# OSU-Bee-Lab/buzzdetect

Hardware: AMD Instinct MI355X
Metric: yamnet_windows_per_s (higher is better)
Workload: dtype f32 (split-f16x3 MFMA products, f32 accumulate)

## Files before the change

### buzzdetect_amd/csrc/bd_device.h

```cpp
#pragma once

#include "bd_internal.h"

#include <mutex>
#include <type_traits>
#ifdef BD_KERNEL_TRACE
#include <cstdio>
#include <cstdlib>
#endif

namespace bd {

namespace {

typedef float f32x16 __attribute__((ext_vector_type(16)));
typedef float v2f __attribute__((ext_vector_type(2)));
typedef float v4f __attribute__((ext_vector_type(4)));
typedef unsigned v4u __attribute__((ext_vector_type(4)));
typedef unsigned u32x2 __attribute__((ext_vector_type(2)));
typedef _Float16 f16x2 __attribute__((ext_vector_type(2)));
typedef _Float16 f16x4 __attribute__((ext_vector_type(4)));
typedef _Float16 f16x8 __attribute__((ext_vector_type(8)));

constexpr float kF16Max = 65504.0f;
// ... 71 lines not shown
                    }
    return true;
}
static_assert(tr_image_is_bijection(), "every (half, k, chunk) has its own 8 bytes of the slot, and they fill it");
static_assert(tr_image_writes_conflict_free(), "a lane group of the publication meets no bank twice");
static_assert(tr_image_reads_conflict_free(), "a lane half of the transposed read meets no bank twice");
__device__ __forceinline__ int tr_read_lane_off(int lane) {
    const int g = lane >> 4, q = (lane >> 2) & 3, p = lane & 3;
    return tr_image_off(0, tr_read_k(0, g >> 1, 0, q), tr_read_chunk(0, g & 1, p));
}
__host__ __device__ constexpr int tr_read_next(int off) { return (off ^ 16) + 4 * kTrRowBytes; }
constexpr bool tr_read_next_holds() {
    for (int lane = 0; lane < 64; ++lane) {
        const int g = lane >> 4, q = (lane >> 2) & 3, p = lane & 3;
        if (tr_read_next(tr_image_off(0, tr_read_k(0, g >> 1, 0, q), tr_read_chunk(0, g & 1, p))) !=
            tr_image_off(0, tr_read_k(0, g >> 1, 1, q), tr_read_chunk(0, g & 1, p)))
            return false;
        for (int s = 0; s < 2; ++s)
            for (int i = 0; i < 3; ++i)
                for (int r = 0; r < 2; ++r)
                    if (tr_image_off(0, tr_read_k(s, g >> 1, r, q), tr_read_chunk(i, g & 1, p)) !=
                        tr_image_off(0, tr_read_k(0, g >> 1, r, q), tr_read_chunk(0, g & 1, p)) + 16 * s * kTrRowBytes + 64 * i)
                        return false;
    }
    return true;
}
static_assert(tr_read_next_holds(), "the reader's immediates");
__device__ __forceinline__ f16x8 tr_read_frag(const char* p0, const char* p1) {
    typedef short s16x4 __attribute__((ext_vector_type(4)));
    typedef __attribute__((address_space(3))) s16x4* lds4;
    const s16x4 a = __builtin_amdgcn_ds_read_tr16_b64_v4i16((lds4)p0), b = __builtin_amdgcn_ds_read_tr16_b64_v4i16((lds4)p1);
    return __builtin_bit_cast(f16x8, __builtin_shufflevector(a, b, 0, 1, 2, 3, 4, 5, 6, 7));
}

__device__ __forceinline__ unsigned pw_lds_addr(const void* p) {
    return (unsigned)(unsigned long long)(__attribute__((address_space(3))) const void*)p;
}
template <int OFFSET>
__device__ __forceinline__ f16x8 pw_lds_frag(unsigned addr) {
    f16x8 v;
    asm volatile("ds_read_b128 %0, %1 offset:%2" : "=v"(v) : "v"(addr), "n"(OFFSET) : "memory");
    return v;
}
__device__ __forceinline__ void pw_lds_store64(unsigned addr, f16x4 v) {
    asm volatile("ds_write_b64 %0, %1" ::"v"(addr), "v"(v) : "memory");
}
__device__ __forceinline__ f16x8 pw_landed(f16x8 v) {
    asm volatile("" : "+v"(v));
    return v;
}
template <int N>
__device__ __forceinline__ void pw_lds_wait() {
    asm volatile("s_waitcnt lgkmcnt(%0)" ::"n"(N) : "memory");
}
template <int I, int E, typename F>
__device__ __forceinline__ void static_for_pw(F&& f) {
    if constexpr (I < E) {
        f(std::integral_constant<int, I>{});
        static_for_pw<I + 1, E>(f);
    }
}
template <int K16, int V, int R>
struct PwResSchedule {
    static constexpr int split_at(int q) {
        for (int j = 0; j < V; ++j)
            if (q == j * K16 / (V > 0 ? V : 1) + 1) return j;
// ... 59 lines not shown
```

### buzzdetect_amd/csrc/bd_internal.h

```cpp
#pragma once

#include <hip/hip_runtime.h>
#include <stdint.h>

#include <string>
#include <vector>

#include "../../include/buzzdetect_hip.h"

namespace bd {

constexpr int kMelNonZero = 461;

constexpr int kMelStart[BD_MEL_BANDS] = {
    5, 5, 6, 7, 9, 10, 11, 12, 13, 14, 16, 17, 18, 20, 21, 23, 25, 26, 28, 30, 32, 34, 36, 38, 40, 42, 44, 47, 49, 52, 54, 57,
    60, 63, 66, 69, 72, 76, 79, 83, 87, 90, 95, 99, 103, 108, 112, 117, 122, 127, 133, 138, 144, 150, 156, 162, 169, 176, 183,
    190, 198, 206, 214, 223};
constexpr int kMelLen[BD_MEL_BANDS] = {
    1, 2, 3, 3, 2, 2, 2, 2, 3, 3, 2, 3, 3, 3, 4, 3, 3, 4, 4, 4, 4, 4, 4, 4, 4, 5, 5, 5, 5, 5, 6, 6,
    6, 6, 6, 7, 7, 7, 8, 7, 8, 9, 8, 9, 9, 9, 10, 10, 11, 11, 11, 12, 12, 12, 13, 14, 14, 14, 15, 16, 16, 17, 17, 17};
constexpr int mel_offset(int band) {
    int o = 0;
    for (int m = 0; m < band; ++m) o += kMelLen[m];
    return o;
// ... 138 lines not shown
                                  hipStream_t stream);
bool launch_separable_fused_next_dw(const float* in, float* out, int windows, const SepLayer& L, const SepLayer& next,
                                    hipStream_t stream);
void launch_pool_head(const float* act, int windows, const float* head_wt, const float* head_b,
                      int n_classes, float* emb, float* logits, hipStream_t stream);
void launch_head(const float* pooled, int windows, const float* head_wt, const float* head_b, int n_classes,
                 float* logits, hipStream_t stream);

void launch_pointwise_res(const float* in, float* out, int rows, const SepLayer& L, hipStream_t stream);
void launch_pointwise_sep_ws(const float* in, float* out, int64_t rows, const SepLayer& L, hipStream_t stream);
bool launch_sep_ws_next_dw(const float* in, float* out, int windows, const SepLayer& L, const SepLayer& next, hipStream_t stream);

bool launch_l4_window_next_dw(const float* in, float* out, int windows, const SepLayer& L, const SepLayer& next, hipStream_t stream);
bool l4_window_planes_supported(const SepLayer& L3, const SepLayer& L4, const SepLayer& L5);
bool launch_l4_window_planes(const void* planes, const SepLayer& L3, const SepLayer& L4, const SepLayer& L5, float* out,
                             int windows, hipStream_t stream);

void launch_stem4(const float* logmel, int patch_step, const WindowMap& map, int w0, int windows, const float* c1_w,
                  const float* c1_b,
                  const SepLayer& L2, const SepLayer& L3, float* out, hipStream_t stream);

void launch_stem_reg(const float* logmel, int patch_step, const WindowMap& map, int w0, int windows, const float* c1_w,
                     const float* c1_b, const SepLayer& L2, const SepLayer& L3, float* out, hipStream_t stream);
void launch_stem_reg_planes(const float* logmel, int patch_step, const WindowMap& map, int w0, int windows, const float* c1_w,
                            const float* c1_b, const SepLayer& L2, const SepLayer& L3, float* out, hipStream_t stream);

void launch_stem_reg_f32(const float* logmel, int patch_step, const WindowMap& map, int w0, int windows, const float* c1_w,
                         const float* c1_b, const SepLayer& L2, const SepLayer& L3, float* out, hipStream_t stream);

bool launch_l4_reg_f32(const float* in, float* out, int windows, const SepLayer& L4, const SepLayer& L5, hipStream_t stream);

bool launch_separable_mid(const float* in, float* out, int windows, const SepLayer& L5, const SepLayer& L6, const SepLayer& L7,
                          hipStream_t stream);
constexpr int kDw7PlaneBytes = 8 * 2 * 24 * 32 * 2;
bool separable_mid_planes_supported(const SepLayer& L5, const SepLayer& L6, const SepLayer& L7);
bool launch_separable_mid_planes(const float* in, void* out, int windows, const SepLayer& L5, const SepLayer& L6, const SepLayer& L7,
                                 hipStream_t stream);

bool launch_separable_mid_f32(const float* in, float* out, int windows, const SepLayer& L5, const SepLayer& L6, const SepLayer& L7,
                              hipStream_t stream);

bool separable_chip_pw7_supported(const SepLayer& L7, const SepLayer* L, int nl, const SepLayer& next, int windows);
bool launch_separable_chip_pw7(const void* in, float* out, int windows, const SepLayer& L7, const SepLayer* L, int nl,
                               const SepLayer& next, hipStream_t stream);
int launch_separable_run_next_dw(const float* a, float* b, int windows, const SepLayer* L, int max_layers, hipStream_t stream,
                                 bool planes = false);

bool launch_separable_chip_f32(const float* in, float* out, int windows, const SepLayer* L, int nl, hipStream_t stream,
                               const SepLayer* next, bool dw0_done);

bool tail_supported(const SepLayer& L13, const SepLayer& L14);
bool launch_tail_pw13_dw14(const void* in, void* out, int windows, const SepLayer& L13, const SepLayer& L14, hipStream_t stream);
bool launch_tail_pw14_pool(const void* in, float* pooled, int windows, const SepLayer& L14, hipStream_t stream);
bool tail_f32_supported(const SepLayer& L13, const SepLayer& L14);
bool launch_tail_f32(const float* in, float* mid, float* pooled, int windows, const SepLayer& L13, const SepLayer& L14, hipStream_t stream,
                     int which);

struct DenseLayer {
    int k, n;
    int act;
    const float* wfrag;
    const float* bias;
};
size_t dense_packed_floats(int k, int n);
void dense_pack_weights(const float* kernel, int k, int n, float* dst);
void launch_dense(const float* A, int lda, int windows, const DenseLayer& L, float* C, int ldc, hipStream_t stream);
void launch_softmax_rows(const float* x, int ldx, float* y, int windows, int n, hipStream_t stream);
// ... 52 lines not shown
```

### buzzdetect_amd/csrc/sepchip.hip

```cpp
#include "bd_device.h"

namespace bd {

namespace {

constexpr int kChipHalfBytes = 97 * 64;
constexpr int kChipSlotBytes = 2 * kChipHalfBytes;

constexpr int kChipMaxLayers = 5;
struct ChipChain {
    const float* dw_w[kChipMaxLayers];
    const float* dw_b[kChipMaxLayers];
    const _Float16* whi[kChipMaxLayers];
    const _Float16* wlo[kChipMaxLayers];
    const float* pw_u[kChipMaxLayers];
    const float* pw_b[kChipMaxLayers];
    const float* ndw_w;
    const _Float16 *w7hi, *w7lo;
    const float *u7, *b7;
};
template <typename T>
__device__ __forceinline__ const T* chain_ptr(int field, int li) {
    typedef const __attribute__((address_space(4))) unsigned long long* kptr;
    const kptr ka = (kptr)__builtin_amdgcn_kernarg_segment_ptr();
    return reinterpret_cast<const T*>(ka[field * kChipMaxLayers + li]);
}
static_assert(sizeof(ChipChain) == (6 * kChipMaxLayers + 5) * 8, "six tables of five pointers + five");

template <bool PLAIN, int NSLOT, bool TRACE = false, bool NDW = false, bool PLANES = false, bool PW7 = false>
__global__ __launch_bounds__(512, 2) void sep_chip_kernel(const ChipChain ch, const float* X, float* Y, int nl,
                                                           long long M, unsigned* __restrict__ range_flag,
                                                           unsigned long long* __restrict__ dbg = nullptr, int tune = 0) {
    static_assert(NSLOT >= 9 && NSLOT <= 16, "ring size");
    constexpr int K = 512, KQ = K / 16;
    constexpr int NPEND = 16 - NSLOT;
    extern __shared__ __attribute__((aligned(16))) char sm[];
    const int tid = threadIdx.x;
    const int lane = tid & 63;
    const int wc = __builtin_amdgcn_readfirstlane(tid >> 6);
    const int frow = lane & 31, fh = lane >> 5;
    const long long m0 = (long long)blockIdx.x * 96;
    float rmax = 0.0f;
    int tsn = 0;
#define CHIP_TS()                                                                                         \
    if constexpr (TRACE) {                                                                                \
        if (blockIdx.x == 0 && lane == 0 && (wc == 0 || wc == 5) && tsn < 64)                             \
            dbg[(wc == 5 ? 64 : 0) + tsn] = __builtin_amdgcn_s_memtime();                                 \
        ++tsn;                                                                                            \
    }
    CHIP_TS()

    const int wk0 = ((frow >> 1) & 7) << 3;
    const int ra0 = frow * 64 + ((fh ^ ((frow >> 2) & 3)) << 4);
    const int ra1 = ra0 + 2048 + (frow >= 16 ? 64 : 0);
    const int rt0 = tr_read_lane_off(lane), rt1 = tr_read_next(rt0);
    const unsigned lane16 = lane * 16, c4 = frow * 4;

    f32x16 acc[3][2];
    unsigned pend[48], out0[48];

#define CHIP_DW(J, ST, TAPS)                                                                              \
    {                                                                                                     \
        float wt[9];                                                                                      \
        _Pragma("unroll") for (int t = 0; t < 9; ++t)                                                     \
            wt[t] = __builtin_bit_cast(float, __builtin_amdgcn_raw_buffer_load_b32(TAPS, c4, (t * K + 32 * (ST)) * 4, 0)); \
        const float shift = __builtin_bit_cast(float, __builtin_amdgcn_raw_buffer_load_b32(TAPS, c4, (9 * K + 32 * (ST)) * 4, 0)); \
        _Pragma("unroll") for (int y = 0; y < 6; ++y)                                                     \
            _Pragma("unroll") for (int xp = 0; xp < 2; ++xp) {                                            \
                v2f a[2];                                                                                 \
                _Pragma("unroll") for (int d = 0; d < 2; ++d) {                                           \
                    const int x = 2 * xp + d;                                                             \
                    a[d] = v2f{shift, shift};                                                             \
                    _Pragma("unroll") for (int kh = 0; kh < 3; ++kh)                                      \
                        _Pragma("unroll") for (int kw = 0; kw < 3; ++kw) {                                \
                            const int iy = y + kh - 1, ix = x + kw - 1;                                   \
                            if (iy < 0 || iy >= 6 || ix < 0 || ix >= 4) continue;                         \
                            a[d] = __builtin_elementwise_fma(in2[iy][ix], v2f{wt[kh * 3 + kw], wt[kh * 3 + kw]}, a[d]); \
                        }                                                                                 \
                }                                                                                         \
                _Pragma("unroll") for (int w = 0; w < 2; ++w) {                                           \
                    const float v0 = fmaxf(w ? a[0].y : a[0].x, 0.0f), v1 = fmaxf(w ? a[1].y : a[1].x, 0.0f); \
                    const f16x2 h_ = {(_Float16)v0, (_Float16)v1};     \
                    const unsigned hi_ = __builtin_bit_cast(unsigned, h_);                                \
                    unsigned lo_;                                                                         \
                     \
                     \
                    asm volatile("v_fma_mixlo_f16 %0, %2, -1.0, %3 op_sel:[0,0,0] op_sel_hi:[1,0,0]\n\t"  \
                                 "v_fma_mixhi_f16 %0, %2, -1.0, %4 op_sel:[1,0,0] op_sel_hi:[1,0,0]\n\t"  \
                                 "v_max_f32 %1, %1, %3\n\tv_max_f32 %1, %1, %4"                           \
                                 : "=&v"(lo_), "+v"(rmax) : "v"(hi_), "v"(v0), "v"(v1));                  \
                    const int ci = 2 * (6 * w + y) + xp;     \
                    if ((J) == 1) { pend[ci] = hi_; pend[24 + ci] = lo_; }                                \
                    else { out0[ci] = hi_; out0[24 + ci] = lo_; }                                         \
                }                                                                                         \
            }                                                                                             \
    }
#define CHIP_PUBLISH()                                                                                    \
    {                                                                                                     \
        int wkl = wk0;        \
        asm volatile("" : "+v"(wkl));                             \
        char* const slot0 = sm + wc * kChipSlotBytes + frow * kTrRowBytes;                                \
        _Pragma("unroll") for (int j = 0; j < 12; ++j) CHIP_PUT(slot0, j, out0)                           \
        if (wc + 8 < NSLOT) {                                                \
            char* const slot1 = sm + (wc + 8) * kChipSlotBytes + frow * kTrRowBytes;                      \
            _Pragma("unroll") for (int j = 0; j < 12; ++j) CHIP_PUT(slot1, j, pend)                       \
        }                                                                                                 \
    }
#define CHIP_PUT(ROW, J, PK)                                                                              \
    {                                                                                                     \
        char* const p_ = (ROW) + ((96 * fh + 8 * (J)) ^ wkl);                                             \
        *reinterpret_cast<u32x2*>(p_) = u32x2{PK[2 * (J)], PK[2 * (J) + 1]};                              \
        *reinterpret_cast<u32x2*>(p_ + kTrHalfBytes) = u32x2{PK[24 + 2 * (J)], PK[25 + 2 * (J)]};         \
    }
#define CHIP_TAPS_RSRC(DW_W) __builtin_amdgcn_make_buffer_rsrc(const_cast<float*>(DW_W), 0, 10 * K * 4, 0x00020000)

    auto k_loop = [&](auto kq_c, auto row_c, const _Float16* const Wfhi, const _Float16* const Wflo) __attribute__((always_inline)) {
        constexpr int KQL = decltype(kq_c)::value;
        constexpr bool ROWIMG = decltype(row_c)::value;
        constexpr int NS = KQL / 2;
        constexpr int NP = NS > NSLOT ? NS - NSLOT : 0;
        static_assert(NP == 0 || NP == NPEND, "a layer of K = 512 or one that fits the ring");
        const __amdgpu_buffer_rsrc_t bhr = __builtin_amdgcn_make_buffer_rsrc(const_cast<_Float16*>(Wfhi), 0, 16 * KQL * K * 2, 0x00020000);
        const __amdgpu_buffer_rsrc_t blr = __builtin_amdgcn_make_buffer_rsrc(const_cast<_Float16*>(Wflo), 0, 16 * KQL * K * 2, 0x00020000);
        const int btile = wc * (KQL * 1024);
        constexpr int jstep = 8 * KQL * 1024;
        f16x8 bh0[2], bl0[2], bh1[2], bl1[2];
#define CHIP_LB(R, B, Q, J) B[J] = __builtin_bit_cast(f16x8, __builtin_amdgcn_raw_buffer_load_b128(R, lane16, btile + (J) * jstep + (Q) * 1024, 0));
#define CHIP_BLOAD(BH, BL, Q) { CHIP_LB(bhr, BH, Q, 0) CHIP_LB(blr, BL, Q, 0) CHIP_LB(bhr, BH, Q, 1) CHIP_LB(blr, BL, Q, 1) }
        CHIP_BLOAD(bh0, bl0, 0)
        __syncthreads();
        CHIP_TS()

        float zero;
        asm volatile("v_mov_b32 %0, 0" : "=v"(zero));
#pragma unroll
        for (int i = 0; i < 3; ++i)
#pragma unroll
            for (int j = 0; j < 2; ++j)
#pragma unroll
                for (int r = 0; r < 16; ++r) acc[i][j][r] = zero;
#define CHIP_LAH(A, S, I) A = *reinterpret_cast<const f16x8*>(abase + (((I) == 1 ? ra1 : ra0) ^ ((S) << 5)) + ((I) == 2 ? 4096 + 64 : 0));
#define CHIP_LAL(A, S, I) A = *reinterpret_cast<const f16x8*>(abase + (((I) == 1 ? ra1 : ra0) ^ ((S) << 5)) + ((I) == 2 ? 4096 + 64 : 0) + kChipHalfBytes);
#define CHIP_MF(I, J, A, B) acc[I][J] = __builtin_amdgcn_mfma_f32_32x32x16_f16(A, B, acc[I][J], 0, 0, 0);
#define CHIP_SB __builtin_amdgcn_sched_barrier(0);
#define CHIP_NOP
#define CHIP_STEP(I, AH, AL, BH, BL, M1, M2, M3, M4, M5, M6)                                              \
    if constexpr (!PLAIN) {                                                                               \
        CHIP_MF(I, 0, AL, BH[0]) M1 CHIP_SB                                                               \
        CHIP_MF(I, 0, AH, BL[0]) M2 CHIP_SB                                                               \
    } else {                                                                                              \
        M1 M2                                                                                             \
    }                                                                                                     \
    CHIP_MF(I, 0, AH, BH[0]) M3 CHIP_SB                                                                   \
    if constexpr (!PLAIN) {                                                                               \
        CHIP_MF(I, 1, AL, BH[1]) M4 CHIP_SB                                                               \
        CHIP_MF(I, 1, AH, BL[1]) M5 CHIP_SB                                                               \
    } else {                                                                                              \
        M4 M5                                                                                             \
    }                                                                                                     \
    CHIP_MF(I, 1, AH, BH[1]) M6 CHIP_SB
#define CHIP_STAGES_ROW(FROM, TO)                                                                           \
    if ((FROM) < (TO)) {                                                                                  \
        f16x8 ah0, al0, ah1, al1, ah2, al2;                                                               \
        const char* abase = sm + ((FROM) < NSLOT ? (FROM) : (FROM) - NSLOT) * kChipSlotBytes;             \
        CHIP_LAH(ah0, 0, 0) CHIP_LAL(al0, 0, 0) CHIP_LAH(ah1, 0, 1) CHIP_LAL(al1, 0, 1)                   \
        _Pragma("nounroll") for (int kk = (FROM); kk < (TO); ++kk) {                                      \
            const int q1 = 2 * kk + 1, q2 = 2 * kk + 2 < KQL ? 2 * kk + 2 : 0;     \
            const char* const anext = sm + (kk + 1 < (TO) ? (kk + 1 < NSLOT ? kk + 1 : kk + 1 - NSLOT) : (kk < NSLOT ? kk : kk - NSLOT)) * kChipSlotBytes; \
            CHIP_STEP(0, ah0, al0, bh0, bl0, CHIP_LB(bhr, bh1, q1, 0), CHIP_LB(blr, bl1, q1, 0), CHIP_LB(bhr, bh1, q1, 1),  \
                      CHIP_LB(blr, bl1, q1, 1), CHIP_LAH(ah2, 0, 2), CHIP_LAL(al2, 0, 2))                 \
            CHIP_STEP(1, ah1, al1, bh0, bl0, CHIP_LAH(ah0, 1, 0), CHIP_LAL(al0, 1, 0), CHIP_NOP, CHIP_NOP, CHIP_NOP, CHIP_NOP) \
            CHIP_STEP(2, ah2, al2, bh0, bl0, CHIP_LAH(ah1, 1, 1), CHIP_LAL(al1, 1, 1), CHIP_LB(blr, bl0, q2, 0),            \
                      CHIP_LB(bhr, bh0, q2, 0), CHIP_NOP, CHIP_LB(blr, bl0, q2, 1))                       \
            CHIP_STEP(0, ah0, al0, bh1, bl1, CHIP_LB(bhr, bh0, q2, 1), CHIP_LAH(ah2, 1, 2), CHIP_LAL(al2, 1, 2), CHIP_NOP, CHIP_NOP, CHIP_NOP) \
            abase = anext;          \
            CHIP_STEP(1, ah1, al1, bh1, bl1, CHIP_LAH(ah0, 0, 0), CHIP_LAL(al0, 0, 0), CHIP_NOP, CHIP_NOP, CHIP_NOP, CHIP_NOP) \
            CHIP_STEP(2, ah2, al2, bh1, bl1, CHIP_LAH(ah1, 0, 1), CHIP_LAL(al1, 0, 1), CHIP_NOP, CHIP_NOP, CHIP_NOP, CHIP_NOP) \
        }                                                                                                 \
    }
#define CHIP_TR(V, HALF, S, I, R)                                                                         \
    V = __builtin_amdgcn_ds_read_tr16_b64_v4i16((lds4)(abase + ((R) ? rt1 : rt0) + 64 * (I) + 16 * kTrRowBytes * (S) + (HALF) * kTrHalfBytes));
#define CHIP_FR(A, B) __builtin_bit_cast(f16x8, __builtin_shufflevector(A, B, 0, 1, 2, 3, 4, 5, 6, 7))
#define CHIP_STAGES_TR(FROM, TO)                                                                          \
    if ((FROM) < (TO)) {                                                                                  \
        s16x4 h0a, h0b, l0a, l0b, h1a, h1b, l1a, l1b, h2a, h2b, l2a, l2b;                                 \
        const char* abase = sm + ((FROM) < NSLOT ? (FROM) : (FROM) - NSLOT) * kChipSlotBytes;             \
        CHIP_TR(l0a, 1, 0, 0, 0) CHIP_TR(l0b, 1, 0, 0, 1) CHIP_TR(h0a, 0, 0, 0, 0) CHIP_TR(h0b, 0, 0, 0, 1) \
        CHIP_TR(l1a, 1, 0, 1, 0) CHIP_TR(l1b, 1, 0, 1, 1) CHIP_TR(h1a, 0, 0, 1, 0) CHIP_TR(h1b, 0, 0, 1, 1) \
        _Pragma("nounroll") for (int kk = (FROM); kk < (TO); ++kk) {                                      \
            const int q1 = 2 * kk + 1, q2 = 2 * kk + 2 < KQL ? 2 * kk + 2 : 0;     \
            const char* const anext = sm + (kk + 1 < (TO) ? (kk + 1 < NSLOT ? kk + 1 : kk + 1 - NSLOT) : (kk < NSLOT ? kk : kk - NSLOT)) * kChipSlotBytes; \
            CHIP_STEP(0, CHIP_FR(h0a, h0b), CHIP_FR(l0a, l0b), bh0, bl0, CHIP_LB(bhr, bh1, q1, 0), CHIP_LB(blr, bl1, q1, 0),     \
                      CHIP_LB(bhr, bh1, q1, 1), CHIP_LB(blr, bl1, q1, 1), CHIP_TR(l2a, 1, 0, 2, 0), CHIP_TR(l2b, 1, 0, 2, 1))    \
            CHIP_STEP(1, CHIP_FR(h1a, h1b), CHIP_FR(l1a, l1b), bh0, bl0, CHIP_TR(h2a, 0, 0, 2, 0), CHIP_TR(h2b, 0, 0, 2, 1),     \
                      CHIP_TR(l0a, 1, 1, 0, 0), CHIP_TR(l0b, 1, 1, 0, 1), CHIP_TR(h0a, 0, 1, 0, 0), CHIP_TR(h0b, 0, 1, 0, 1))    \
            CHIP_STEP(2, CHIP_FR(h2a, h2b), CHIP_FR(l2a, l2b), bh0, bl0, CHIP_TR(l1a, 1, 1, 1, 0), CHIP_TR(l1b, 1, 1, 1, 1),     \
                      CHIP_LB(blr, bl0, q2, 0), CHIP_LB(bhr, bh0, q2, 0), CHIP_TR(h1a, 0, 1, 1, 0), CHIP_LB(blr, bl0, q2, 1))    \
            CHIP_STEP(0, CHIP_FR(h0a, h0b), CHIP_FR(l0a, l0b), bh1, bl1, CHIP_LB(bhr, bh0, q2, 1), CHIP_TR(h1b, 0, 1, 1, 1),     \
                      CHIP_TR(l2a, 1, 1, 2, 0), CHIP_TR(l2b, 1, 1, 2, 1), CHIP_TR(h2a, 0, 1, 2, 0), CHIP_TR(h2b, 0, 1, 2, 1))    \
            abase = anext;          \
            CHIP_STEP(1, CHIP_FR(h1a, h1b), CHIP_FR(l1a, l1b), bh1, bl1, CHIP_TR(l0a, 1, 0, 0, 0), CHIP_TR(l0b, 1, 0, 0, 1),     \
                      CHIP_TR(h0a, 0, 0, 0, 0), CHIP_TR(h0b, 0, 0, 0, 1), CHIP_NOP, CHIP_NOP)                                   \
            CHIP_STEP(2, CHIP_FR(h2a, h2b), CHIP_FR(l2a, l2b), bh1, bl1, CHIP_TR(l1a, 1, 0, 1, 0), CHIP_TR(l1b, 1, 0, 1, 1),     \
                      CHIP_TR(h1a, 0, 0, 1, 0), CHIP_TR(h1b, 0, 0, 1, 1), CHIP_NOP, CHIP_NOP)                                   \
        }                                                                                                 \
    }
#define CHIP_STAGES(FROM, TO)                                                                             \
    if constexpr (ROWIMG) {                                                                               \
        CHIP_STAGES_ROW(FROM, TO)                                                                         \
    } else {                                                                                              \
        CHIP_STAGES_TR(FROM, TO)                                                                          \
    }
        typedef short s16x4 __attribute__((ext_vector_type(4)));
        typedef __attribute__((address_space(3))) s16x4* lds4;
        CHIP_STAGES(0, NP)
        CHIP_TS()
        if constexpr (NP > 0) {
            __syncthreads();
            CHIP_TS()
            if (wc >= 8 - NPEND) {
                char* const slot = sm + (wc + 8 - NSLOT) * kChipSlotBytes + frow * kTrRowBytes;
                int wkl = wk0;
                asm volatile("" : "+v"(wkl));
#pragma unroll
                for (int j = 0; j < 12; ++j) CHIP_PUT(slot, j, pend)
            }
        }
        CHIP_TS()
        if constexpr (NP > 0) __syncthreads();
        CHIP_TS()
        CHIP_STAGES(NP, NS)
        CHIP_TS()
#undef CHIP_STAGES
#undef CHIP_STAGES_ROW
#undef CHIP_STAGES_TR
#undef CHIP_TR
#undef CHIP_FR
#undef CHIP_STEP
#undef CHIP_BLOAD
#undef CHIP_LB
#undef CHIP_LAH
#undef CHIP_LAL
#undef CHIP_MF
#undef CHIP_SB
#undef CHIP_NOP
    };

    auto next_layer = [&](const float* const taps_w, const float* const pu, const float* const pb) __attribute__((always_inline)) {
        const __amdgpu_buffer_rsrc_t taps = CHIP_TAPS_RSRC(taps_w);
        const __amdgpu_buffer_rsrc_t pur = __builtin_amdgcn_make_buffer_rsrc(const_cast<float*>(pu), 0, K * 4, 0x00020000);
        const __amdgpu_buffer_rsrc_t pbr = __builtin_amdgcn_make_buffer_rsrc(const_cast<float*>(pb), 0, K * 4, 0x00020000);
        if (wc >= 4) __syncthreads();
#pragma unroll
        for (int j = 0; j < 2; ++j) {
            const int st = j ? wc + 8 : wc;
            const float u = __builtin_bit_cast(float, __builtin_amdgcn_raw_buffer_load_b32(pur, c4, 128 * st, 0));
            const float b = __builtin_bit_cast(float, __builtin_amdgcn_raw_buffer_load_b32(pbr, c4, 128 * st, 0));
            float ev[12][4];
#pragma unroll
            for (int q = 0; q < 6; ++q)
#pragma unroll
                for (int x = 0; x < 4; ++x) {
                    const float a01 = fmaxf(fmaf(acc[q >> 2][j][4 * (q & 3) + x], u, b), 0.0f);
                    const float a23 = fmaxf(fmaf(acc[(q + 6) >> 2][j][4 * ((q + 6) & 3) + x], u, b), 0.0f);
                    const auto r = __builtin_amdgcn_permlane32_swap(__builtin_bit_cast(unsigned, a01),
                                                                    __builtin_bit_cast(unsigned, a23), false, false);
                    ev[2 * q][x] = __builtin_bit_cast(float, (unsigned)r[0]);
                    ev[2 * q + 1][x] = __builtin_bit_cast(float, (unsigned)r[1]);
                }
            v2f in2[6][4];
#pragma unroll
            for (int y = 0; y < 6; ++y)
#pragma unroll
                for (int x = 0; x < 4; ++x) in2[y][x] = v2f{ev[y][x], ev[6 + y][x]};
            if (j == 0) CHIP_DW(0, st, taps)
            else CHIP_DW(1, st, taps)
            CHIP_TS()
        }
        if (wc < 4) __syncthreads();
        CHIP_TS()
        CHIP_PUBLISH()
    };

    const long long rows_left = M - m0;
    const unsigned tile_bytes = (unsigned)(rows_left < 96 ? rows_left : 96) * (K * 4);
    if constexpr (PW7) {
        const long long w0 = m0 / 24, wleft = M / 24 - w0;
        const __amdgpu_buffer_rsrc_t pr = __builtin_amdgcn_make_buffer_rsrc(
            const_cast<char*>(reinterpret_cast<const char*>(X)) + (size_t)w0 * kDw7PlaneBytes, 0,
            (unsigned)(wleft < 4 ? wleft : 4) * kDw7PlaneBytes, 0x00020000);
        constexpr int kPieces = 8 * kChipSlotBytes / 1024;
        static_assert(kPieces * 1024 == 8 * kChipSlotBytes && 8 * kChipSlotBytes <= NSLOT * kChipSlotBytes, "whole pieces");
#pragma unroll
        for (int t = 0; t < (kPieces + 7) / 8; ++t) {
            const int n = 8 * t + wc;
            if (n >= kPieces) break;
            const int c = 64 * n + lane;
            const int s = c / (kChipSlotBytes / 16), cs = c - s * (kChipSlotBytes / 16);
            const int h = cs >= kChipHalfBytes / 16 ? 1 : 0;
            const int o = (cs - h * (kChipHalfBytes / 16)) * 16;
            const bool skew = o >= 48 * 64 && o < 49 * 64;
            const int rho = o < 48 * 64 ? o >> 6 : (o - 64) >> 6;
            const int p = (o >> 4) & 3, w = rho / 24;
            const unsigned src = (unsigned)(w * kDw7PlaneBytes + s * (kDw7PlaneBytes / 8) + h * (kDw7PlaneBytes / 16) +
                                            (rho - 24 * w) * 64 + ((p ^ ((rho >> 2) & 3)) << 4));
            const unsigned off = skew || (PLAIN && h) ? 0x7ffffff0u : src;
            __builtin_amdgcn_raw_ptr_buffer_load_lds(pr, (__attribute__((address_space(3))) void*)(sm + n * 1024), 16, off, 0, 0, 0);
        }
        asm volatile("s_waitcnt vmcnt(0)" ::: "memory");
        CHIP_TS()
        k_loop(std::integral_constant<int, 16>{}, std::true_type{}, ch.w7hi, ch.w7lo);
        next_layer(ch.dw_w[0], ch.u7, ch.b7);
    } else {
        const __amdgpu_buffer_rsrc_t xrs = __builtin_amdgcn_make_buffer_rsrc(const_cast<float*>(X) + (size_t)m0 * K, 0, tile_bytes, 0x00020000);
        const __amdgpu_buffer_rsrc_t taps0 = CHIP_TAPS_RSRC(ch.dw_w[0]);
        const unsigned xo = (48u * fh * K) * 4 + c4;
#pragma unroll
        for (int j = 0; j < 2; ++j) {
            const int st = j ? wc + 8 : wc;
            v2f in2[6][4];
#pragma unroll
            for (int y = 0; y < 6; ++y)
#pragma unroll
                for (int x = 0; x < 4; ++x) {
                    in2[y][x].x = __builtin_bit_cast(float, __builtin_amdgcn_raw_buffer_load_b32(xrs, xo, ((4 * y + x) * K + 32 * st) * 4, 0));
                    in2[y][x].y = __builtin_bit_cast(float, __builtin_amdgcn_raw_buffer_load_b32(xrs, xo, ((24 + 4 * y + x) * K + 32 * st) * 4, 0));
                }
            if (j == 0) CHIP_DW(0, st, taps0)
            else CHIP_DW(1, st, taps0)
            CHIP_TS()
            __builtin_amdgcn_sched_barrier(0);
        }
        CHIP_PUBLISH()
    }

    for (int li = 0; li < nl; ++li) {
        k_loop(std::integral_constant<int, KQ>{}, std::false_type{}, chain_ptr<_Float16>(2, li), chain_ptr<_Float16>(3, li));
        if (li + 1 == nl) break;
        next_layer(chain_ptr<float>(0, li + 1), chain_ptr<float>(4, li), chain_ptr<float>(5, li));
    }
#undef CHIP_DW
#undef CHIP_PUBLISH
#undef CHIP_TAPS_RSRC
#undef CHIP_PUT

    {
        const __amdgpu_buffer_rsrc_t pur = __builtin_amdgcn_make_buffer_rsrc(const_cast<float*>(chain_ptr<float>(4, nl - 1)), 0, K * 4, 0x00020000);
        const __amdgpu_buffer_rsrc_t pbr = __builtin_amdgcn_make_buffer_rsrc(const_cast<float*>(chain_ptr<float>(5, nl - 1)), 0, K * 4, 0x00020000);
        if constexpr (!NDW) {
            const __amdgpu_buffer_rsrc_t yrs = __builtin_amdgcn_make_buffer_rsrc(Y + (size_t)m0 * K, 0, tile_bytes, 0x00020000);
            const unsigned yo = (4u * fh * K) * 4 + c4;
#pragma unroll
            for (int j = 0; j < 2; ++j) {
                const int st = j ? wc + 8 : wc;
                const float u = __builtin_bit_cast(float, __builtin_amdgcn_raw_buffer_load_b32(pur, c4, 128 * st, 0));
                const float b = __builtin_bit_cast(float, __builtin_amdgcn_raw_buffer_load_b32(pbr, c4, 128 * st, 0));
#pragma unroll
                for (int i = 0; i < 3; ++i)
#pragma unroll
                    for (int r = 0; r < 16; ++r)
                        __builtin_amdgcn_raw_buffer_store_b32(__builtin_bit_cast(unsigned, fmaxf(fmaf(acc[i][j][r], u, b), 0.0f)), yrs, yo,
                                                              ((32 * i + 8 * (r >> 2) + (r & 3)) * K + 32 * st) * 4, 0);
            }
        } else {
            const __amdgpu_buffer_rsrc_t yrs = __builtin_amdgcn_make_buffer_rsrc(Y + (size_t)(m0 / 4) * K, 0, tile_bytes / 4, 0x00020000);
            _Float16* const yh = reinterpret_cast<_Float16*>(Y);
            const __amdgpu_buffer_rsrc_t yhr = __builtin_amdgcn_make_buffer_rsrc(yh + (size_t)(m0 / 4) * K, 0, tile_bytes / 8, 0x00020000);
            const __amdgpu_buffer_rsrc_t ylr = __builtin_amdgcn_make_buffer_rsrc(yh + (size_t)(M / 4 + m0 / 4) * K, 0, tile_bytes / 8, 0x00020000);
            const __amdgpu_buffer_rsrc_t ntaps = __builtin_amdgcn_make_buffer_rsrc(const_cast<float*>(ch.ndw_w), 0, 10 * K * 4, 0x00020000);
            const unsigned yo = (12u * fh * K) * 4 + c4;
// ... 166 lines not shown
```

### buzzdetect_amd/csrc/sepmid.hip

```cpp
#include "bd_device.h"

#include <type_traits>

namespace bd {

namespace {

constexpr int kHalfA = 97 * 64;
constexpr int kSlotA = 2 * kHalfA;
constexpr int kHalf7 = 48 * 64;
constexpr int kSlot7 = 2 * kHalf7;
constexpr int kOffA7 = 8 * kSlotA;
constexpr int kMidLds = kOffA7 + 8 * kSlot7 + 1024;
static_assert(kMidLds <= 160 * 1024, "one workgroup per CU");
constexpr int kStage7 = kDw7PlaneBytes / 8;
constexpr int kMidLdsDw7 = kOffA7 + 8 * kStage7;
static_assert(kStage7 == 2 * 24 * 64, "[hi, lo][24 rows][32 channels] f16");

struct MidArgs {
    const _Float16 *w5h, *w5l, *w6h, *w6l, *w7h, *w7l;
    const float *u5, *b5, *u6, *b6, *u7, *b7;
    const float *dw6, *dw7;
};

#define MID_RSRC(P, BYTES) __builtin_amdgcn_make_buffer_rsrc(const_cast<void*>(static_cast<const void*>(P)), 0, (BYTES), 0x00020000)
#define MID_LD32(R, VOFF, SOFF) __builtin_bit_cast(float, __builtin_amdgcn_raw_buffer_load_b32(R, VOFF, SOFF, 0))
#define MID_LD128(R, VOFF, SOFF) __builtin_bit_cast(f16x8, __builtin_amdgcn_raw_buffer_load_b128(R, VOFF, SOFF, 0))

template <bool PLAIN, bool TRACE, bool DW7OUT = false>
__global__ __launch_bounds__(512, 2) void sep_mid_kernel(const MidArgs a, const float* __restrict__ X, float* __restrict__ Y, int windows,
                                                          unsigned* __restrict__ range_flag, unsigned long long* __restrict__ dbg) {
    extern __shared__ __attribute__((aligned(16))) char sm[];
    const int tid = threadIdx.x, lane = tid & 63;
    const int wc = __builtin_amdgcn_readfirstlane(tid >> 6);
    const int frow = lane & 31, fh = lane >> 5;
    float rmax = 0.0f;
    int tsn = 0;
#define MID_TS()                                                                                          \
    if constexpr (TRACE) {                                                                                \
        if (blockIdx.x == 0 && lane == 0 && (wc == 0 || wc == 5) && tsn < 64)                             \
            dbg[(wc == 5 ? 64 : 0) + tsn] = __builtin_amdgcn_s_memtime();                                 \
        ++tsn;                                                                                            \
    }
    const int wb5 = (frow >> 3) * kSlotA + fh * 64 + (((frow & 7) >> 1) << 4) + 8 * (frow & 1);
    static_assert((kSlotA & 0x70) == 0 && kHalfA % 8 == 0, "the slot bits of wb5 are its own; 8-byte writes");
    const int wb7 = fh * 128 + ((frow >> 3) << 4) + 2 * (frow & 7);
    const int ra0 = frow * 64 + ((fh ^ ((frow >> 2) & 3)) << 4);
    const int ra1 = ra0 + 2048 + (frow >= 16 ? 64 : 0);
    const int wt6 = ((frow >> 1) & 7) << 3;
    const int rt0 = tr_read_lane_off(lane), rt1 = tr_read_next(rt0);
// ... 166 lines not shown
#pragma unroll
        for (int i = 0; i < 3; ++i)
#pragma unroll
            for (int r = 0; r < 16; ++r) acc[i][r] = zero;
        {
            constexpr int KQ = 16;
#pragma unroll
            for (int q = 0; q < KQ; ++q) {
                if (q + 2 < KQ) {
                    bh[(q + 2) % 3] = MID_LD128(r6h, lane16, (wc * KQ + q + 2) * 1024);
                    bl[(q + 2) % 3] = MID_LD128(r6l, lane16, (wc * KQ + q + 2) * 1024);
                }
                const char* const ab = sm + (q >> 1) * kSlotA + (q & 1) * 16 * kTrRowBytes;
#pragma unroll
                for (int i = 0; i < 3; ++i) {
                    const f16x8 ah = tr_read_frag(ab + rt0 + 64 * i, ab + rt1 + 64 * i);
                    const f16x8 al = tr_read_frag(ab + rt0 + 64 * i + kTrHalfBytes, ab + rt1 + 64 * i + kTrHalfBytes);
                    MID_MMA(acc[i], ah, al, bh[q % 3], bl[q % 3])
                }
            }
        }
        MID_TS()
        if (win_next >= 0) fetch_window(win_next);
        {
            const __amdgpu_buffer_rsrc_t ur = MID_RSRC(a.u6, 1024), br = MID_RSRC(a.b6, 1024), tr = MID_RSRC(a.dw7, 10 * 256 * 4);
            const float u = MID_LD32(ur, c4, 128 * wc), b = MID_LD32(br, c4, 128 * wc);
            float wt[9];
#pragma unroll
            for (int t = 0; t < 9; ++t) wt[t] = MID_LD32(tr, c4, (t * 256 + 32 * wc) * 4);
            const float shift = MID_LD32(tr, c4, (9 * 256 + 32 * wc) * 4);
            float ev[12][4], lh[12], rh[12];
            MID_TILE_TO_MAP(acc, u, b, ev)
            MID_HALO(ev, lh, rh)
            int wbl = wb7;
            asm volatile("" : "+v"(wbl));
            char* const slot = sm + kOffA7 + wc * kSlot7;
            char* const stg = sm + kOffA7 + wc * kStage7;
            v2f in2[8][6];
            MID_ROW_PAIRS(ev, lh, rh, in2)
#pragma unroll
            for (int oy = 0; oy < 3; ++oy)
#pragma unroll
                for (int j = 0; j < 2; ++j) {
                    v2f sacc = {shift, shift};
#pragma unroll
                    for (int kh = 0; kh < 3; ++kh)
#pragma unroll
                        for (int kw = 0; kw < 3; ++kw)
                            sacc = __builtin_elementwise_fma(in2[1 + 2 * oy + kh][1 + 2 * j + kw], v2f{wt[kh * 3 + kw], wt[kh * 3 + kw]}, sacc);
#pragma unroll
                    for (int w = 0; w < 2; ++w) {
                        const int oyw = oy + 3 * w;
                        const float o = fmaxf(w ? sacc.y : sacc.x, 0.0f);
                        MID_SPLIT(o, pk)
                        if constexpr (DW7OUT) {
                            char* const p_ = stg + (4 * oyw + 2 * fh + j) * 64 + 2 * frow;
                            *reinterpret_cast<unsigned short*>(p_) = (unsigned short)pk;
                            if constexpr (!PLAIN) *reinterpret_cast<unsigned short*>(p_ + kStage7 / 2) = (unsigned short)(pk >> 16);
                        } else {
                            char* const p_ = slot + (wbl ^ (((6 * HALF + oyw) & 3) << 4)) + (24 * HALF + 4 * oyw + j) * 64;
                            *reinterpret_cast<unsigned short*>(p_) = (unsigned short)pk;
                            *reinterpret_cast<unsigned short*>(p_ + kHalf7) = (unsigned short)(pk >> 16);
                        }
                    }
                }
            if constexpr (DW7OUT) {
                typedef __attribute__((address_space(1))) char* gchar;
                asm volatile("" ::: "memory");
                const gchar dst = (gchar)Y + (size_t)win * kDw7PlaneBytes + wc * kStage7 + lane * 16;
#pragma unroll
                for (int t = 0; t < 3; ++t) {
                    if (PLAIN && (t == 2 || (t == 1 && lane >= 32))) continue;
                    const v4f v = *reinterpret_cast<const v4f*>(stg + t * 1024 + lane * 16);
                    asm volatile("global_store_dwordx4 %0, %1, off\n\ts_nop 2" : : "v"(dst + t * 1024), "v"(v) : "memory");
                }
            }
        }
        if constexpr (LAST) {
#pragma unroll
            for (int q = 0; q < 2; ++q)
#pragma unroll
                for (int j = 0; j < 2; ++j) {
                    b7h[q][j] = MID_LD128(r7h, lane16, ((wc + 8 * j) * 16 + q) * 1024);
                    b7l[q][j] = MID_LD128(r7l, lane16, ((wc + 8 * j) * 16 + q) * 1024);
                }
        }
        __syncthreads();
        MID_TS()
    };
    auto layer7 = [&](auto nw_c, int win) {
        constexpr int NW = decltype(nw_c)::value;
        f32x16 c7[NW][2];
        float zero;
        asm volatile("v_mov_b32 %0, 0" : "=v"(zero));
#pragma unroll
        for (int i = 0; i < NW; ++i)
#pragma unroll
            for (int j = 0; j < 2; ++j)
#pragma unroll
                for (int r = 0; r < 16; ++r) c7[i][j][r] = zero;
        constexpr int KQ = 16;
        const int ra7 = frow * 64 + ((fh ^ ((frow >> 2) & 3)) << 4);
#pragma unroll
        for (int q = 0; q < KQ; ++q) {
            if (q + 2 < KQ) {
#pragma unroll
                for (int j = 0; j < 2; ++j) {
                    b7h[(q + 2) % 3][j] = MID_LD128(r7h, lane16, ((wc + 8 * j) * KQ + q + 2) * 1024);
// ... 120 lines not shown
```

Before: 2.098 million.

## Store dw7 planes channel-major from registers and DMA them into transposed-read layout

Changes the dw7 intermediate plane layout to channel-major with 24 contiguous positions per channel. The producer packs pairs with permlane32_swap and stores straight from registers, dropping the LDS staging buffer. The chip kernel's LDS-DMA loader now places those planes into the transposed-read slot layout, so the row-image A-read path can be removed and the ds_read_tr path reused. Compile-time checks prove the mapping is a bijection and free of bank conflicts. The cost is more global store instructions per lane and a changed inter-kernel layout contract.

```diff
diff --git a/buzzdetect_amd/csrc/bd_device.h b/buzzdetect_amd/csrc/bd_device.h
--- a/buzzdetect_amd/csrc/bd_device.h
+++ b/buzzdetect_amd/csrc/bd_device.h
@@ -127,6 +127,91 @@
     const s16x4 a = __builtin_amdgcn_ds_read_tr16_b64_v4i16((lds4)p0), b = __builtin_amdgcn_ds_read_tr16_b64_v4i16((lds4)p1);
     return __builtin_bit_cast(f16x8, __builtin_shufflevector(a, b, 0, 1, 2, 3, 4, 5, 6, 7));
 }
+
+constexpr int kPlaneChanBytes = 24 * 2, kPlaneHalfBytes = 32 * kPlaneChanBytes, kPlaneStageBytes = 2 * kPlaneHalfBytes;
+static_assert(kDw7PlaneBytes == 8 * kPlaneStageBytes, "eight stages of 32 channels per window");
+__host__ __device__ constexpr int dw7_plane_off(int half, int channel, int pos) {
+    return (channel >> 5) * kPlaneStageBytes + half * kPlaneHalfBytes + (channel & 31) * kPlaneChanBytes + pos * 2;
+}
+__host__ __device__ constexpr int dma_stage_off(int half, int k, int chunk) {
+    return half * kTrHalfBytes + k * kTrRowBytes + (chunk << 3);
+}
+__host__ __device__ constexpr int dma_unit_src(int stage, int unit, int window_bytes) {
+    const int half = unit / 384, k = unit % 384 / 12, U = unit % 12;
+    return U / 3 * window_bytes + dw7_plane_off(half, 32 * stage + k, 8 * (U % 3));
+}
+constexpr bool dma_stage_is_bijection() {
+    constexpr int kWin = 8 * kPlaneStageBytes;
+    bool seen[4 * kWin / 16] = {};
+    for (int s = 0; s < 8; ++s)
+        for (int unit = 0; unit < 768; ++unit) {
+            const int half = unit / 384, k = unit % 384 / 12, U = unit % 12;
+            if (dma_stage_off(half, k, 2 * U) != unit * 16 || dma_stage_off(half, k, 2 * U + 1) != unit * 16 + 8) return false;
+            const int o = dma_unit_src(s, unit, kWin);
+            if (o < 0 || o >= 4 * kWin || o % 16 || seen[o / 16]) return false;
+            for (int e = 0; e < 8; e += 7)
+                if (o + 2 * e != (8 * U + e) / 24 * kWin + dw7_plane_off(half, 32 * s + k, (8 * U + e) % 24)) return false;
+            seen[o / 16] = true;
+        }
+    for (int i = 0; i < 4 * kWin / 16; ++i)
+        if (!seen[i]) return false;
+    return true;
+}
+constexpr bool dma_stage_writes_conflict_free() {
+    for (int piece = 0; piece < kTrSlotBytes / 1024; ++piece)
+        for (int grp = 0; grp < 4; ++grp) {
+            unsigned long long banks = 0;
+            for (int l = 0; l < 16; ++l)
+                for (int d = 0; d < 4; ++d) {
+                    const int unit = 64 * piece + 16 * grp + l;
+                    const unsigned long long b = 1ull << ((dma_stage_off(unit / 384, unit % 384 / 12, 2 * (unit % 12)) / 4 + d) % 64);
+                    if (banks & b) return false;
+                    banks |= b;
+                }
+        }
+    return true;
+}
+constexpr bool dma_stage_reads_conflict_free() {
+    for (int half = 0; half < 2; ++half)
+        for (int i = 0; i < 3; ++i)
+            for (int s = 0; s < 2; ++s)
+                for (int h = 0; h < 2; ++h)
+                    for (int r = 0; r < 2; ++r) {
+                        unsigned long long banks = 0;
+                        for (int gp = 0; gp < 2; ++gp)
+                            for (int q = 0; q < 4; ++q)
+                                for (int p = 0; p < 4; ++p)
+                                    for (int d = 0; d < 2; ++d) {
+                                        const unsigned long long b =
+                                            1ull << ((dma_stage_off(half, tr_read_k(s, h, r, q), tr_read_chunk(i, gp, p)) / 4 + d) % 64);
+                                        if (banks & b) return false;
+                                        banks |= b;
+                                    }
+                    }
+    return true;
+}
+static_assert(dma_stage_is_bijection(), "every 16 bytes of eight stages come from their own 16 bytes of the tile's planes");
+static_assert(dma_stage_writes_conflict_free(), "a lane group of the LDS-DMA meets no bank twice");
+static_assert(dma_stage_reads_conflict_free(), "a lane half of the transposed read meets no bank twice");
+__device__ __forceinline__ int dma_read_lane_off(int lane) {
+    const int g = lane >> 4, q = (lane >> 2) & 3, p = lane & 3;
+    return dma_stage_off(0, tr_read_k(0, g >> 1, 0, q), tr_read_chunk(0, g & 1, p));
+}
+__host__ __device__ constexpr int dma_read_next(int off) { return off + 4 * kTrRowBytes; }
+constexpr bool dma_read_next_holds() {
+    for (int lane = 0; lane < 64; ++lane) {
+        const int g = lane >> 4, q = (lane >> 2) & 3, p = lane & 3;
+        for (int s = 0; s < 2; ++s)
+            for (int i = 0; i < 3; ++i)
+                for (int r = 0; r < 2; ++r)
+                    if (dma_stage_off(0, tr_read_k(s, g >> 1, r, q), tr_read_chunk(i, g & 1, p)) !=
+                        (r ? dma_read_next(dma_stage_off(0, tr_read_k(0, g >> 1, 0, q), tr_read_chunk(0, g & 1, p)))
+                           : dma_stage_off(0, tr_read_k(0, g >> 1, 0, q), tr_read_chunk(0, g & 1, p))) + 16 * s * kTrRowBytes + 64 * i)
+                        return false;
+    }
+    return true;
+}
+static_assert(dma_read_next_holds(), "the reader's immediates");
 
 __device__ __forceinline__ unsigned pw_lds_addr(const void* p) {
     return (unsigned)(unsigned long long)(__attribute__((address_space(3))) const void*)p;
diff --git a/buzzdetect_amd/csrc/bd_internal.h b/buzzdetect_amd/csrc/bd_internal.h
--- a/buzzdetect_amd/csrc/bd_internal.h
+++ b/buzzdetect_amd/csrc/bd_internal.h
@@ -194,7 +194,7 @@
 
 bool launch_separable_mid(const float* in, float* out, int windows, const SepLayer& L5, const SepLayer& L6, const SepLayer& L7,
                           hipStream_t stream);
-constexpr int kDw7PlaneBytes = 8 * 2 * 24 * 32 * 2;
+constexpr int kDw7PlaneBytes = 8 * 2 * 32 * 24 * 2;
 bool separable_mid_planes_supported(const SepLayer& L5, const SepLayer& L6, const SepLayer& L7);
 bool launch_separable_mid_planes(const float* in, void* out, int windows, const SepLayer& L5, const SepLayer& L6, const SepLayer& L7,
                                  hipStream_t stream);
diff --git a/buzzdetect_amd/csrc/sepchip.hip b/buzzdetect_amd/csrc/sepchip.hip
--- a/buzzdetect_amd/csrc/sepchip.hip
+++ b/buzzdetect_amd/csrc/sepchip.hip
@@ -4,8 +4,7 @@
 
 namespace {
 
-constexpr int kChipHalfBytes = 97 * 64;
-constexpr int kChipSlotBytes = 2 * kChipHalfBytes;
+constexpr int kChipSlotBytes = kTrSlotBytes;
 
 constexpr int kChipMaxLayers = 5;
 struct ChipChain {
@@ -51,8 +50,6 @@
     CHIP_TS()
 
     const int wk0 = ((frow >> 1) & 7) << 3;
-    const int ra0 = frow * 64 + ((fh ^ ((frow >> 2) & 3)) << 4);
-    const int ra1 = ra0 + 2048 + (frow >= 16 ? 64 : 0);
     const int rt0 = tr_read_lane_off(lane), rt1 = tr_read_next(rt0);
     const unsigned lane16 = lane * 16, c4 = frow * 4;
 
@@ -114,9 +111,8 @@
     }
 #define CHIP_TAPS_RSRC(DW_W) __builtin_amdgcn_make_buffer_rsrc(const_cast<float*>(DW_W), 0, 10 * K * 4, 0x00020000)
 
-    auto k_loop = [&](auto kq_c, auto row_c, const _Float16* const Wfhi, const _Float16* const Wflo) __attribute__((always_inline)) {
+    auto k_loop = [&](auto kq_c, const int a0, const int a1, const _Float16* const Wfhi, const _Float16* const Wflo) __attribute__((always_inline)) {
         constexpr int KQL = decltype(kq_c)::value;
-        constexpr bool ROWIMG = decltype(row_c)::value;
         constexpr int NS = KQL / 2;
         constexpr int NP = NS > NSLOT ? NS - NSLOT : 0;
         static_assert(NP == 0 || NP == NPEND, "a layer of K = 512 or one that fits the ring");
@@ -139,8 +135,6 @@
             for (int j = 0; j < 2; ++j)
 #pragma unroll
                 for (int r = 0; r < 16; ++r) acc[i][j][r] = zero;
-#define CHIP_LAH(A, S, I) A = *reinterpret_cast<const f16x8*>(abase + (((I) == 1 ? ra1 : ra0) ^ ((S) << 5)) + ((I) == 2 ? 4096 + 64 : 0));
-#define CHIP_LAL(A, S, I) A = *reinterpret_cast<const f16x8*>(abase + (((I) == 1 ? ra1 : ra0) ^ ((S) << 5)) + ((I) == 2 ? 4096 + 64 : 0) + kChipHalfBytes);
 #define CHIP_MF(I, J, A, B) acc[I][J] = __builtin_amdgcn_mfma_f32_32x32x16_f16(A, B, acc[I][J], 0, 0, 0);
 #define CHIP_SB __builtin_amdgcn_sched_barrier(0);
 #define CHIP_NOP
@@ -159,29 +153,10 @@
         M4 M5                                                                                             \
     }                                                                                                     \
     CHIP_MF(I, 1, AH, BH[1]) M6 CHIP_SB
-#define CHIP_STAGES_ROW(FROM, TO)                                                                           \
-    if ((FROM) < (TO)) {                                                                                  \
-        f16x8 ah0, al0, ah1, al1, ah2, al2;                                                               \
-        const char* abase = sm + ((FROM) < NSLOT ? (FROM) : (FROM) - NSLOT) * kChipSlotBytes;             \
-        CHIP_LAH(ah0, 0, 0) CHIP_LAL(al0, 0, 0) CHIP_LAH(ah1, 0, 1) CHIP_LAL(al1, 0, 1)                   \
-        _Pragma("nounroll") for (int kk = (FROM); kk < (TO); ++kk) {                                      \
-            const int q1 = 2 * kk + 1, q2 = 2 * kk + 2 < KQL ? 2 * kk + 2 : 0;     \
-            const char* const anext = sm + (kk + 1 < (TO) ? (kk + 1 < NSLOT ? kk + 1 : kk + 1 - NSLOT) : (kk < NSLOT ? kk : kk - NSLOT)) * kChipSlotBytes; \
-            CHIP_STEP(0, ah0, al0, bh0, bl0, CHIP_LB(bhr, bh1, q1, 0), CHIP_LB(blr, bl1, q1, 0), CHIP_LB(bhr, bh1, q1, 1),  \
-                      CHIP_LB(blr, bl1, q1, 1), CHIP_LAH(ah2, 0, 2), CHIP_LAL(al2, 0, 2))                 \
-            CHIP_STEP(1, ah1, al1, bh0, bl0, CHIP_LAH(ah0, 1, 0), CHIP_LAL(al0, 1, 0), CHIP_NOP, CHIP_NOP, CHIP_NOP, CHIP_NOP) \
-            CHIP_STEP(2, ah2, al2, bh0, bl0, CHIP_LAH(ah1, 1, 1), CHIP_LAL(al1, 1, 1), CHIP_LB(blr, bl0, q2, 0),            \
-                      CHIP_LB(bhr, bh0, q2, 0), CHIP_NOP, CHIP_LB(blr, bl0, q2, 1))                       \
-            CHIP_STEP(0, ah0, al0, bh1, bl1, CHIP_LB(bhr, bh0, q2, 1), CHIP_LAH(ah2, 1, 2), CHIP_LAL(al2, 1, 2), CHIP_NOP, CHIP_NOP, CHIP_NOP) \
-            abase = anext;          \
-            CHIP_STEP(1, ah1, al1, bh1, bl1, CHIP_LAH(ah0, 0, 0), CHIP_LAL(al0, 0, 0), CHIP_NOP, CHIP_NOP, CHIP_NOP, CHIP_NOP) \
-            CHIP_STEP(2, ah2, al2, bh1, bl1, CHIP_LAH(ah1, 0, 1), CHIP_LAL(al1, 0, 1), CHIP_NOP, CHIP_NOP, CHIP_NOP, CHIP_NOP) \
-        }                                                                                                 \
-    }
 #define CHIP_TR(V, HALF, S, I, R)                                                                         \
-    V = __builtin_amdgcn_ds_read_tr16_b64_v4i16((lds4)(abase + ((R) ? rt1 : rt0) + 64 * (I) + 16 * kTrRowBytes * (S) + (HALF) * kTrHalfBytes));
+    V = __builtin_amdgcn_ds_read_tr16_b64_v4i16((lds4)(abase + ((R) ? a1 : a0) + 64 * (I) + 16 * kTrRowBytes * (S) + (HALF) * kTrHalfBytes));
 #define CHIP_FR(A, B) __builtin_bit_cast(f16x8, __builtin_shufflevector(A, B, 0, 1, 2, 3, 4, 5, 6, 7))
-#define CHIP_STAGES_TR(FROM, TO)                                                                          \
+#define CHIP_STAGES(FROM, TO)                                                                             \
     if ((FROM) < (TO)) {                                                                                  \
         s16x4 h0a, h0b, l0a, l0b, h1a, h1b, l1a, l1b, h2a, h2b, l2a, l2b;                                 \
         const char* abase = sm + ((FROM) < NSLOT ? (FROM) : (FROM) - NSLOT) * kChipSlotBytes;             \
@@ -205,12 +180,6 @@
                       CHIP_TR(h1a, 0, 0, 1, 0), CHIP_TR(h1b, 0, 0, 1, 1), CHIP_NOP, CHIP_NOP)                                   \
         }                                                                                                 \
     }
-#define CHIP_STAGES(FROM, TO)                                                                             \
-    if constexpr (ROWIMG) {                                                                               \
-        CHIP_STAGES_ROW(FROM, TO)                                                                         \
-    } else {                                                                                              \
-        CHIP_STAGES_TR(FROM, TO)                                                                          \
-    }
         typedef short s16x4 __attribute__((ext_vector_type(4)));
         typedef __attribute__((address_space(3))) s16x4* lds4;
         CHIP_STAGES(0, NP)
@@ -232,15 +201,11 @@
         CHIP_STAGES(NP, NS)
         CHIP_TS()
 #undef CHIP_STAGES
-#undef CHIP_STAGES_ROW
-#undef CHIP_STAGES_TR
 #undef CHIP_TR
 #undef CHIP_FR
 #undef CHIP_STEP
 #undef CHIP_BLOAD
 #undef CHIP_LB
-#undef CHIP_LAH
-#undef CHIP_LAL
 #undef CHIP_MF
 #undef CHIP_SB
 #undef CHIP_NOP
@@ -290,26 +255,20 @@
             const_cast<char*>(reinterpret_cast<const char*>(X)) + (size_t)w0 * kDw7PlaneBytes, 0,
             (unsigned)(wleft < 4 ? wleft : 4) * kDw7PlaneBytes, 0x00020000);
         constexpr int kPieces = 8 * kChipSlotBytes / 1024;
-        static_assert(kPieces * 1024 == 8 * kChipSlotBytes && 8 * kChipSlotBytes <= NSLOT * kChipSlotBytes, "whole pieces");
-#pragma unroll
-        for (int t = 0; t < (kPieces + 7) / 8; ++t) {
+        static_assert(kPieces * 1024 == 8 * kChipSlotBytes && kPieces % 8 == 0 && 8 <= NSLOT, "whole pieces, as many per wave");
+#pragma unroll
+        for (int t = 0; t < kPieces / 8; ++t) {
             const int n = 8 * t + wc;
-            if (n >= kPieces) break;
             const int c = 64 * n + lane;
             const int s = c / (kChipSlotBytes / 16), cs = c - s * (kChipSlotBytes / 16);
-            const int h = cs >= kChipHalfBytes / 16 ? 1 : 0;
-            const int o = (cs - h * (kChipHalfBytes / 16)) * 16;
-            const bool skew = o >= 48 * 64 && o < 49 * 64;
-            const int rho = o < 48 * 64 ? o >> 6 : (o - 64) >> 6;
-            const int p = (o >> 4) & 3, w = rho / 24;
-            const unsigned src = (unsigned)(w * kDw7PlaneBytes + s * (kDw7PlaneBytes / 8) + h * (kDw7PlaneBytes / 16) +
-                                            (rho - 24 * w) * 64 + ((p ^ ((rho >> 2) & 3)) << 4));
-            const unsigned off = skew || (PLAIN && h) ? 0x7ffffff0u : src;
+            const bool lo = cs >= kTrHalfBytes / 16;
+            const unsigned off = PLAIN && lo ? 0x7ffffff0u : (unsigned)dma_unit_src(s, cs, kDw7PlaneBytes);
             __builtin_amdgcn_raw_ptr_buffer_load_lds(pr, (__attribute__((address_space(3))) void*)(sm + n * 1024), 16, off, 0, 0, 0);
         }
         asm volatile("s_waitcnt vmcnt(0)" ::: "memory");
         CHIP_TS()
-        k_loop(std::integral_constant<int, 16>{}, std::true_type{}, ch.w7hi, ch.w7lo);
+        const int rd0 = dma_read_lane_off(lane);
+        k_loop(std::integral_constant<int, 16>{}, rd0, dma_read_next(rd0), ch.w7hi, ch.w7lo);
         next_layer(ch.dw_w[0], ch.u7, ch.b7);
     } else {
         const __amdgpu_buffer_rsrc_t xrs = __builtin_amdgcn_make_buffer_rsrc(const_cast<float*>(X) + (size_t)m0 * K, 0, tile_bytes, 0x00020000);
@@ -335,7 +294,7 @@
     }
 
     for (int li = 0; li < nl; ++li) {
-        k_loop(std::integral_constant<int, KQ>{}, std::false_type{}, chain_ptr<_Float16>(2, li), chain_ptr<_Float16>(3, li));
+        k_loop(std::integral_constant<int, KQ>{}, rt0, rt1, chain_ptr<_Float16>(2, li), chain_ptr<_Float16>(3, li));
         if (li + 1 == nl) break;
         next_layer(chain_ptr<float>(0, li + 1), chain_ptr<float>(4, li), chain_ptr<float>(5, li));
     }
diff --git a/buzzdetect_amd/csrc/sepmid.hip b/buzzdetect_amd/csrc/sepmid.hip
--- a/buzzdetect_amd/csrc/sepmid.hip
+++ b/buzzdetect_amd/csrc/sepmid.hip
@@ -13,9 +13,7 @@
 constexpr int kOffA7 = 8 * kSlotA;
 constexpr int kMidLds = kOffA7 + 8 * kSlot7 + 1024;
 static_assert(kMidLds <= 160 * 1024, "one workgroup per CU");
-constexpr int kStage7 = kDw7PlaneBytes / 8;
-constexpr int kMidLdsDw7 = kOffA7 + 8 * kStage7;
-static_assert(kStage7 == 2 * 24 * 64, "[hi, lo][24 rows][32 channels] f16");
+constexpr int kMidLdsDw7 = kOffA7;
 
 struct MidArgs {
     const _Float16 *w5h, *w5l, *w6h, *w6l, *w7h, *w7l;
@@ -248,48 +246,75 @@
             float ev[12][4], lh[12], rh[12];
             MID_TILE_TO_MAP(acc, u, b, ev)
             MID_HALO(ev, lh, rh)
-            int wbl = wb7;
-            asm volatile("" : "+v"(wbl));
-            char* const slot = sm + kOffA7 + wc * kSlot7;
-            char* const stg = sm + kOffA7 + wc * kStage7;
             v2f in2[8][6];
             MID_ROW_PAIRS(ev, lh, rh, in2)
-#pragma unroll
-            for (int oy = 0; oy < 3; ++oy)
-#pragma unroll
-                for (int j = 0; j < 2; ++j) {
-                    v2f sacc = {shift, shift};
-#pragma unroll
-                    for (int kh = 0; kh < 3; ++kh)
-#pragma unroll
-                        for (int kw = 0; kw < 3; ++kw)
-                            sacc = __builtin_elementwise_fma(in2[1 + 2 * oy + kh][1 + 2 * j + kw], v2f{wt[kh * 3 + kw], wt[kh * 3 + kw]}, sacc);
+            if constexpr (DW7OUT) {
+                unsigned h7[6], l7[6];
+#pragma unroll
+                for (int oy = 0; oy < 3; ++oy) {
+                    v2f sacc[2];
+#pragma unroll
+                    for (int j = 0; j < 2; ++j) {
+                        sacc[j] = v2f{shift, shift};
+#pragma unroll
+                        for (int kh = 0; kh < 3; ++kh)
+#pragma unroll
+                            for (int kw = 0; kw < 3; ++kw)
+                                sacc[j] = __builtin_elementwise_fma(in2[1 + 2 * oy + kh][1 + 2 * j + kw], v2f{wt[kh * 3 + kw], wt[kh * 3 + kw]}, sacc[j]);
+                    }
 #pragma unroll
                     for (int w = 0; w < 2; ++w) {
-                        const int oyw = oy + 3 * w;
-                        const float o = fmaxf(w ? sacc.y : sacc.x, 0.0f);
-                        MID_SPLIT(o, pk)
-                        if constexpr (DW7OUT) {
-                            char* const p_ = stg + (4 * oyw + 2 * fh + j) * 64 + 2 * frow;
-                            *reinterpret_cast<unsigned short*>(p_) = (unsigned short)pk;
-                            if constexpr (!PLAIN) *reinterpret_cast<unsigned short*>(p_ + kStage7 / 2) = (unsigned short)(pk >> 16);
-                        } else {
+                        const float o0 = fmaxf(w ? sacc[0].y : sacc[0].x, 0.0f), o1 = fmaxf(w ? sacc[1].y : sacc[1].x, 0.0f);
+                        MID_SPLIT2(o0, o1, h7[oy + 3 * w], l7[oy + 3 * w])
+                    }
+                }
+                unsigned ph[3], qh[3], pl[3], ql[3];
+#pragma unroll
+                for (int e = 0; e < 3; ++e) {
+                    const auto rh_ = __builtin_amdgcn_permlane32_swap(h7[e], h7[e + 3], false, false);
+                    ph[e] = (unsigned)rh_[0];
+                    qh[e] = (unsigned)rh_[1];
+                    if constexpr (!PLAIN) {
+                        const auto rl_ = __builtin_amdgcn_permlane32_swap(l7[e], l7[e + 3], false, false);
+                        pl[e] = (unsigned)rl_[0];
+                        ql[e] = (unsigned)rl_[1];
+                    }
+                }
+                typedef __attribute__((address_space(1))) char* gchar;
+                const gchar dst = (gchar)Y + (size_t)win * kDw7PlaneBytes + dw7_plane_off(0, 32 * wc, 0) + frow * kPlaneChanBytes + fh * 24;
+                static_assert(dw7_plane_off(0, 33, 12) - dw7_plane_off(0, 32, 0) == kPlaneChanBytes + 24 && dw7_plane_off(1, 0, 0) == kPlaneHalfBytes,
+                              "a lane's twelve positions are 24 contiguous bytes of its channel");
+                asm volatile("global_store_dwordx4 %0, %1, off\n\ts_nop 2" : : "v"(dst), "v"(v4u{ph[0], qh[0], ph[1], qh[1]}) : "memory");
+                asm volatile("global_store_dwordx2 %0, %1, off offset:16" : : "v"(dst), "v"(u32x2{ph[2], qh[2]}) : "memory");
+                if constexpr (!PLAIN) {
+                    asm volatile("global_store_dwordx4 %0, %1, off offset:%2\n\ts_nop 2"
+                                 : : "v"(dst), "v"(v4u{pl[0], ql[0], pl[1], ql[1]}), "n"(kPlaneHalfBytes) : "memory");
+                    asm volatile("global_store_dwordx2 %0, %1, off offset:%2" : : "v"(dst), "v"(u32x2{pl[2], ql[2]}), "n"(kPlaneHalfBytes + 16) : "memory");
+                }
+            } else {
+                int wbl = wb7;
+                asm volatile("" : "+v"(wbl));
+                char* const slot = sm + kOffA7 + wc * kSlot7;
+#pragma unroll
+                for (int oy = 0; oy < 3; ++oy)
+#pragma unroll
+                    for (int j = 0; j < 2; ++j) {
+                        v2f sacc = {shift, shift};
+#pragma unroll
+                        for (int kh = 0; kh < 3; ++kh)
+#pragma unroll
+                            for (int kw = 0; kw < 3; ++kw)
+                                sacc = __builtin_elementwise_fma(in2[1 + 2 * oy + kh][1 + 2 * j + kw], v2f{wt[kh * 3 + kw], wt[kh * 3 + kw]}, sacc);
+#pragma unroll
+                        for (int w = 0; w < 2; ++w) {
+                            const int oyw = oy + 3 * w;
+                            const float o = fmaxf(w ? sacc.y : sacc.x, 0.0f);
+                            MID_SPLIT(o, pk)
                             char* const p_ = slot + (wbl ^ (((6 * HALF + oyw) & 3) << 4)) + (24 * HALF + 4 * oyw + j) * 64;
                             *reinterpret_cast<unsigned short*>(p_) = (unsigned short)pk;
                             *reinterpret_cast<unsigned short*>(p_ + kHalf7) = (unsigned short)(pk >> 16);
                         }
                     }
-                }
-            if constexpr (DW7OUT) {
-                typedef __attribute__((address_space(1))) char* gchar;
-                asm volatile("" ::: "memory");
-                const gchar dst = (gchar)Y + (size_t)win * kDw7PlaneBytes + wc * kStage7 + lane * 16;
-#pragma unroll
-                for (int t = 0; t < 3; ++t) {
-                    if (PLAIN && (t == 2 || (t == 1 && lane >= 32))) continue;
-                    const v4f v = *reinterpret_cast<const v4f*>(stg + t * 1024 + lane * 16);
-                    asm volatile("global_store_dwordx4 %0, %1, off\n\ts_nop 2" : : "v"(dst + t * 1024), "v"(v) : "memory");
-                }
             }
         }
         if constexpr (LAST) {
```

Measured after the change: 2.095 million (median of 2 runs). About the same (-0.1%).
